# haberdashPI/SignalOperators.jl

Hardware: AMD Instinct MI355X
Metric: frames/sec sink() 44.1kHz 8ch Mix+Filt+Resample; achieved HBM GB/s (higher is better)
Workload: dtype f64

## Files before the change

signaloperators.jl_amd/csrc/executor.cpp:

```cpp
#include "plan_impl.h"

namespace so {

static inline int carrier_vec_ok(const DCarrier& c, int64_t V) {
    if (!std::getenv("SIGOPS_STRICT_ALIGN")) return (uintptr_t)c.base % (c.dtype == SO_F64 ? 8 : 4) == 0;
    return ((uintptr_t)c.base % 16 == 0) && (c.cstride % V == 0);
}

static hipError_t h2d_small(void* dst, const void* src, size_t bytes) {
    constexpr size_t kPiece = 16 * 1024;
    if (bytes < 2 * kPiece || bytes > (1u << 20)) return hipMemcpy(dst, src, bytes, hipMemcpyHostToDevice);
    for (size_t off = 0; off < bytes; off += kPiece) {
        const hipError_t e = hipMemcpy((char*)dst + off, (const char*)src + off, std::min(kPiece, bytes - off), hipMemcpyHostToDevice);
        if (e != hipSuccess) return e;
    }
    return hipSuccess;
}

static void upload_tables(Plan* P) {
    std::vector<Buf>& bufs = P->bufs;
    auto up = [&](int buf, const auto& v, size_t at = 0) {
        HIPCHECK(h2d_small((char*)bufs[buf].d + at, v.data(), v.size() * sizeof(*v.data())));
    };
    auto alloc_up = [](auto*& d, const auto& v) {
// ... 474 lines not shown
    g.src_has_omega = F.flag;
    g.src_df = F.df;
    g.src_omega = F.v0;
    g.src_phi = F.v1;
    g.src_fs = F.v2;
    const double step = 6.283185307179586476925 * (F.flag ? F.v0 / F.v2 : 1.0 / F.v2);
    g.src_cd = std::cos(step);
    g.src_sd = std::sin(step);
}
static RsGlobalTables global_tables(Plan* P, const Stage& S) {
    return RsGlobalTables{(const RsCtl*)P->bufs[S.ctl_buf].d, (const DCarrier*)P->bufs[S.car_buf].d, P->d_ops, P->d_leaves};
}
static void set_rsos_fixup(RsFixup& F, Plan* P, const Stage& S, const RsosItem& I) {
    F.g = I.g;
    F.tab = I.tab;
    F.jend = I.jend;
    F.jrel = (const int*)P->bufs[S.rsos_jrel_buf].d;
    F.taps = S.rsos_taps;
    F.cf = S.groups[0];
    F.gsrc = I.gsrc;
    F.y = I.y;
}
static void arm_bad(void* words, size_t n, hipStream_t st) { HIPCHECK((hipError_t)launch_fill_u32(words, n, 0x7f7f7f7fu, st)); }

static std::vector<long long> read_trace(const long long* d_trace, size_t trace_n, hipStream_t st, long long& t0) {
    std::vector<long long> tr(trace_n);
    HIPCHECK(hipStreamSynchronize(st));
    HIPCHECK(hipMemcpy(tr.data(), d_trace, trace_n * 8, hipMemcpyDeviceToHost));
    t0 = 0;
    for (size_t i = 0; i < trace_n; ++i)
        if (tr[i] && (!t0 || tr[i] < t0)) t0 = tr[i];
    return tr;
}
static void dump_rs_trace(const long long* d_trace, size_t trace_n, const RsPeriodic& rp, hipStream_t st) {
    long long t0;
    const std::vector<long long> tr = read_trace(d_trace, trace_n, st, t0);
    for (int w = 0; w < rp.nwaves; ++w)
        for (int it = 0; it < kRsTraceIters; ++it) {
            const long long* q = &tr[((size_t)w * kRsTraceIters + it) * kRsTraceStamps];
            if (!q[0]) continue;
            std::fprintf(stderr, "[rs-trace] %s w%02d it%02d", w < rp.ncompute ? "C" : "L", w, it);
            for (int k = 0; k < kRsTraceStamps; ++k) std::fprintf(stderr, " %lld", q[k] ? q[k] - t0 : -1);
            std::fprintf(stderr, "\n");
        }
}
static void dump_rsos_trace(const long long* d_trace, size_t trace_n, const RsSos& rs, hipStream_t st) {
    long long t0;
    const std::vector<long long> tr = read_trace(d_trace, trace_n, st, t0);
    const bool counters = std::atoi(std::getenv("SIGOPS_RSOS_TRACE")) == 2;
    for (int w = 0; w < rs.nwaves; ++w)
        for (int it = 0; it < (counters ? 5 : kRsosTraceIters); ++it) {
            const long long* q = &tr[((size_t)w * kRsosTraceIters + it) * 8];
            if (counters) {
                bool any = false;
                for (int k = 0; k < 8; ++k) any = any || q[k];
                if (!any) continue;
                std::fprintf(stderr, "[rsos-count] w%02d row%d", w, it);
                for (int k = 0; k < 8; ++k) std::fprintf(stderr, " %lld", q[k] - 1);
            } else {
                if (!q[0] && !q[2]) continue;
                std::fprintf(stderr, "[rsos-trace] %s w%02d it%02d", w == 0 ? "C" : (w & 3) == 0 ? "L" : "Y", w, it);
                for (int k = 0; k < 8; ++k) std::fprintf(stderr, " %lld", q[k] ? q[k] - t0 : -1);
            }
            std::fprintf(stderr, "\n");
        }
}


static int run_pointwise(Plan* P, const Step& s, void* outp, hipStream_t st) {
    const PwStep& w = P->pw[s.idx];
    if (w.nblocks <= 0) return 0;
    static const int il_scalar = std::getenv("SIGOPS_K1_ILSCALAR") ? 1 : 0;
    OutView ov{};
    if (w.out_buf >= 0) {
        const Buf& b = P->bufs[w.out_buf];
        ov = OutView{b.d, 1, b.pitch, b.dtype, il_scalar};
    } else if (P->out.is_device) {
        ov = OutView{outp, P->out.frame_stride, P->out.chan_stride, P->out.dtype, il_scalar};
    } else {
        const Buf& b = P->bufs[P->out_stage_buf];
        ov = OutView{b.d, P->interleaved_host ? P->out.nch : 1, P->interleaved_host ? 1 : b.pitch, b.dtype, il_scalar};
    }
    if (w.fill)
        launch_randn_fill(P->d_pieces + w.piece0, w.npieces, w.nblocks, P->d_leaves, ov, st);
    else if (w.rtc) {
        if (rtc_launch(w.rtc, w.nblocks, P->d_pieces + w.piece0, w.npieces, P->d_leaves, ov, st) != 0)
            fail(SO_ERR_RUNTIME, "hipRTC kernel launch failed");
    } else
// ... 251 lines not shown
    a.back = N.nd.l0;
    a.ahead = N.nd.l1;
    a.tab = S.aux_buf >= 0 ? (double*)P->bufs[S.aux_buf].d : nullptr;
    a.nch = N.nch;
    a.op = N.nd.i0;
    const int nl = launch_movsum(a, st);
    if (nl < 0) fail(SO_ERR_UNSUPPORTED, "Movsum: more than 65535 channels, or 2^31 tiles of 2048 frames or blocks of 1024 frames and more, are not lowered");
    return nl;
}

static int run_rsos_fused(Plan* P, const Stage& S, const SosGeom& g, const View& out, hipStream_t st) {
    const Node& N = P->nodes[S.node];
    const Stage& S3 = P->stages[S.rsos_src];
    RsSos rs = S.rs;
    rs.out_pitch = out.pitch;
    rs.out_f32 = g.out_dtype == SO_F32 || N.dtype == SO_F32;
    if (rs.f32m && rs.out_f32) rs.ring32 = 1;
    else rs.f32m = 0;
    rs.sring = rs.f32m && (rs.fuse == 1 || rs.fuse == 2) && !std::getenv("SIGOPS_RSOS_NO_SRING") ? 1 : 0;
    char* const yk = out.d - (size_t)S.rs.store_lo * (rs.out_f32 ? 4 : 8);
    rs.store_lo = S.rs.store_lo + g.store_lo;
    rs.mats = (const double*)P->bufs[S.rsos_mats_buf].d;
    rs.bad = nullptr;
    if (S.bad_buf >= 0 && rs.nranges >= 1 && !std::getenv("SIGOPS_SOS_NOPOISON")) {
        rs.bad = (int32_t*)P->bufs[S.bad_buf].d;
        arm_bad(rs.bad, (size_t)N.nch, st);
    }
    rs.err = kernel_error_word(P);
    static long long* d_rtrace = nullptr;
    static int rtrace_seen = 0;
    const char* const rtrace_skip = std::getenv("SIGOPS_RSOS_TRACE_SKIP");
    const bool rtracing = std::getenv("SIGOPS_RSOS_TRACE") != nullptr && rtrace_seen++ >= (rtrace_skip ? std::atoi(rtrace_skip) : 0);
    const size_t rtrace_n = (size_t)16 * kRsosTraceIters * 8;
    if (rtracing) {
        if (!d_rtrace) HIPCHECK(hipMalloc(&d_rtrace, rtrace_n * 8));
        HIPCHECK(hipMemsetAsync(d_rtrace, 0, rtrace_n * 8, st));
        rs.trace = d_rtrace;
    }
    const double* rtab = (const double*)P->bufs[S.rsos_tab_buf >= 0 ? S.rsos_tab_buf : S3.tab_buf].d;
    const int* rjend = (const int*)P->bufs[S.rsos_jend_buf >= 0 ? S.rsos_jend_buf : S3.jend_buf].d;
    if (launch_rsos(rtab, rjend, rs, yk, global_tables(P, S3), S.rsos_grid, st) != 0)
        fail(SO_ERR_RUNTIME, "internal: no fused resampler + IIR instantiation for this geometry");
    if (rtracing) dump_rsos_trace(d_rtrace, rtrace_n, rs, st);
    int nl = 1;
    if (rs.bad && S.rsos_jrel_buf >= 0 && !std::getenv("SIGOPS_RSOS_NO_FIXUP")) {
        RsFixup fx{};
        set_rsos_fixup(fx, P, S, RsosItem{rs, rtab, rjend, yk, global_tables(P, S3)});
        nl += launch_rsos_fixup(fx, st);
    } else if (rs.bad) {
        SosGeom pg = g;
        pg.n = rs.n_out;
        pg.chunk = rs.pr * rs.L;
        pg.nchunks = rs.nranges;
        pg.store_lo = rs.store_lo;
        pg.bad = rs.bad;
        nl += launch_sos_poison(yk, pg, st);
    }
    return nl;
}

static int run_sos(Plan* P, const Step& s, void* outp, hipStream_t st) {
    const Stage& S = P->stages[s.idx];
    const Node& N = P->nodes[S.node];
    const size_t esz = dsize(N.dtype);
    const View in = stage_in(P, S, N.nch, N.dtype), out = stage_out(P, s.idx, outp);
    SosGeom g = S.sg;
    g.in_pitch = in.pitch;
    g.out_pitch = out.pitch;
    g.store_lo = s.idx == P->alias_stage ? P->alias_skip : 0;
    if (s.idx == P->alias_stage && P->alias_narrow) g.out_dtype = SO_F32;
    g.align_rows = S.pre_stage < 0 && !std::getenv("SIGOPS_SOS_NOALIGN");
// ... 277 lines not shown
        if (!P->out.is_device && P->out.nframes > 0) {
            std::string why;
            if (kernel_gave_up(P, why)) fail(SO_ERR_RUNTIME, why);
        }
        if (P->profiling == 2) P->prof_execs++;
        if (P->profiling == 1) {
            HIPCHECK(hipStreamSynchronize(st));
            double total = 0, best = -1;
            for (size_t si = 0; si < P->steps.size(); ++si) {
                float ms = 0;
                HIPCHECK(hipEventElapsedTime(&ms, P->events[2 * si], P->events[2 * si + 1]));
                P->steps[si].ms = ms;
                total += ms;
                if (ms > best) {
                    best = ms;
                    P->stats.dominant_kernel_ms = ms;
                    P->stats.dominant_kernel_bytes = P->steps[si].bytes;
                    std::snprintf(P->stats.dominant_kernel, sizeof P->stats.dominant_kernel, "%s", P->steps[si].name.c_str());
                }
            }
            P->stats.last_exec_ms = total;
        }
    } catch (const PlanError& e) {
        err = e.msg;
        return e.status;
    }
    return SO_OK;
}

int plan_execute(Plan* P, void* outp, void* stream, std::string& err) {
    DeviceGuard guard(P->device);
    if (kernel_gave_up(P, err)) return SO_ERR_RUNTIME;
    const bool eligible = P->steps.size() >= 4 && P->out.is_device && P->host_leaves.empty() && !P->profiling &&
                          !std::getenv("SIGOPS_NO_GRAPH") && !std::getenv("SIGOPS_RS_TRACE");
    if (!eligible) {
        P->n_direct++;
        return plan_execute_direct(P, outp, stream, err);
    }
    hipStream_t st = (hipStream_t)stream;
    const bool leaves_match = P->out_alias_buf < 0 || P->bufs[P->out_alias_buf].d == outp;
    if (P->graph_exec && P->graph_out == outp && P->graph_epoch == P->array_epoch && leaves_match) {
        if (hipSetDevice(P->device) == hipSuccess && hipGraphLaunch(P->graph_exec, st) == hipSuccess) {
            P->n_replays++;
            return SO_OK;
        }
        (void)hipGetLastError();
        (void)hipGraphExecDestroy(P->graph_exec);
        P->graph_exec = nullptr;
        P->graph_failed = true;
    }
    if (P->graph_failed || P->last_out != outp || P->last_epoch != P->array_epoch) {
        P->last_out = outp;
        P->last_epoch = P->array_epoch;
        P->n_direct++;
        return plan_execute_direct(P, outp, stream, err);
    }
    if (P->graph_exec && P->graph_out == outp && P->graph_epoch == P->array_epoch) {
// ... 175 lines not shown
```

signaloperators.jl_amd/csrc/k_exact.hip:

```cpp
#include "kcommon.h"
#include "kstage.h"

namespace so {

constexpr int kFixThreads = 256;
constexpr int kFixSeg = 1024;
constexpr int kFixIn = 6144;
constexpr int kFixAhead = 64;

template <typename TO>
__device__ __forceinline__ void rsos_fixup_body(const RsFixup& fx) {
    const RsSos& g = fx.g;
    const int ch = blockIdx.y;
    if (ch >= g.nch) return;
    const int r = g.bad[ch];
    if (r < 0 || r >= g.nranges) return;
    TO* const y = (TO*)fx.y + (int64_t)ch * g.out_pitch;
    const int64_t prL = g.pr * g.L;
    const double nan = __longlong_as_double(0x7ff8000000000000ll);
    {
        int64_t f0 = (int64_t)(r + 1) * prL;
        if (f0 < g.store_lo) f0 = g.store_lo;
        for (int64_t f = f0 + (int64_t)blockIdx.x * kFixThreads + threadIdx.x; f < g.n_out; f += (int64_t)gridDim.x * kFixThreads) y[f] = (TO)nan;
    }
    if (blockIdx.x != 0) return;
    __shared__ long long s_first;
    __shared__ double xin[kFixIn];
    __shared__ double xs[kFixSeg];
    __shared__ double ys[kFixAhead + 16];
    const int tid = threadIdx.x;
    const int64_t lo = max((int64_t)r * prL, g.store_lo), hi = min((int64_t)(r + 1) * prL, g.n_out);
    if (tid == 0) s_first = hi;
    __syncthreads();
    for (int64_t m = lo + tid; m < hi; m += kFixThreads)
        if (!isfinite((double)y[m])) {
            atomicMin(&s_first, (long long)m);
            break;
// ... 161 lines not shown
```

signaloperators.jl_amd/csrc/k_rsos.hip:

```cpp
#include "kcommon.h"
#include "kstage.h"

#ifndef SO_RSOS_ONLY_KS
#define SO_RSOS_ONLY_KS -1
#endif
#ifndef SO_RSOS_ONLY_F32
#define SO_RSOS_ONLY_F32 0
#endif
#ifndef SO_RSOS_ONLY_NW
#define SO_RSOS_ONLY_NW 0
#endif

namespace so {

typedef double v4d __attribute__((ext_vector_type(4)));
typedef float v4f __attribute__((ext_vector_type(4)));

#define SO_LDS __attribute__((address_space(3)))
__device__ __forceinline__ int flag_ld(uint32_t a) { return *(const volatile SO_LDS int*)(uintptr_t)a; }
__device__ __forceinline__ void flag_st(uint32_t a, int v) { *(volatile SO_LDS int*)(uintptr_t)a = v; }
#define SO_SPIN_PAUSE(spins, sleep, limit)                         \
    do {                                                           \
        if (++(spins) > (limit)) rsos_wait_failed(sh);             \
        if ((sleep) == 1) __builtin_amdgcn_s_sleep(1);             \
// ... 207 lines not shown
};

__device__ __forceinline__ int uni(int v) { return __builtin_amdgcn_readfirstlane(v); }


#define SO_GLB __attribute__((address_space(1)))

__device__ __forceinline__ void rsos_wait_failed(SO_LDS RsosShared* sh) {
    uint32_t SO_GLB* const e = (uint32_t SO_GLB*)rfl64((int64_t)(uintptr_t)sh->g.err);
    if (e == nullptr) __builtin_trap();
    if ((threadIdx.x & 63) == 0) __hip_atomic_store((uint32_t*)e, 1u, __ATOMIC_RELAXED, __HIP_MEMORY_SCOPE_SYSTEM);
    __threadfence_system();
    asm volatile("s_waitcnt vmcnt(0) lgkmcnt(0)" ::: "memory");
    __builtin_amdgcn_endpgm();
}

#ifndef SO_RSOS_TRACE
#define SO_RSOS_TRACE 0
#endif
__device__ __forceinline__ void rsos_stamp(long long* trace, int wave, int it, int k, int it0 = 400) {
    if constexpr (!SO_RSOS_TRACE) return;
    if (trace != nullptr && blockIdx.x == 0 && (threadIdx.x & 63) == 0 && it >= it0 && it < it0 + kRsosTraceIters)
        ((long long SO_GLB*)trace)[(wave * kRsosTraceIters + (it - it0)) * 8 + k] = clock64();
}

#ifndef SO_RSOS_COUNT
#define SO_RSOS_COUNT 0
#endif
__device__ __forceinline__ void rsos_count_out(long long* trace, int wave, int row, int k, long long v) {
    if constexpr (!SO_RSOS_COUNT) return;
    if (trace != nullptr && blockIdx.x == 0) ((long long SO_GLB*)trace)[((wave * kRsosTraceIters) + row) * 8 + k] = v + 1;
}

struct RsosLds {
    SO_LDS double *taps, *ring, *gtab;
    volatile SO_LDS double *xs, *ss;
    volatile SO_LDS double* xh;
};
__device__ __forceinline__ SO_LDS double* rsos_lds_ptr(const void* p) {
    return (SO_LDS double*)(uintptr_t)__builtin_amdgcn_readfirstlane((uint32_t)(uintptr_t)(const SO_LDS void*)p);
}
#ifndef SO_NSS_EXTRA
#define SO_NSS_EXTRA (ny + 1)
#endif
__host__ __device__ constexpr int rsos_nss(int ny) { return ny + SO_NSS_EXTRA; }
__device__ __forceinline__ RsosLds rsos_carve(double* dyn_, int tapd, int rpitch, int nx, int ns) {
// ... 697 lines not shown
    if (g.store_lo > r0 * g.pr * g.L) return false;
    const int64_t lo_ok = C0.a > 0 ? C0.a : 0, hi_ok = C0.b < g.n_in ? C0.b : g.n_in;
    const int64_t f0 = (r0 * g.pr - g.wp) * g.M + g.wj0, f1 = (r1 * g.pr - g.wp) * g.M + g.wj0 + g.wk;
    return f0 >= lo_ok && f1 <= hi_ok;
}

template <int NY>
__device__ __attribute__((noinline)) void rsos_wproj_y(RsosShared* sh_, double* dyn, int64_t G_, int yi_) {
    constexpr int NX = 2 * NY + 1;
    const int lane = threadIdx.x & 63;
    SO_LDS RsosShared* const sh = (SO_LDS RsosShared*)rsos_lds_ptr(sh_);
    const int64_t G = rfl64(G_);
    const int yi = uni(yi_);
    const SO_LDS RsSos& g = sh->g;
    const RsosLds l = rsos_carve(dyn, uni(g.cyc) > 0 ? 0 : uni(g.ngroups) * uni(g.ks) * 64, uni(g.rpitch), NX, rsos_nss(NY));
    const uint32_t fl_base = (uint32_t)(uintptr_t)sh->flags;
    const int ct = uni(g.ct), K = uni(g.wk);
    const int npairs = (K + 7) >> 3;
    const int c0 = (int)((int64_t)yi * npairs / NY), c1 = (int)((int64_t)(yi + 1) * npairs / NY);
    const double SO_GLB* const V = (const double SO_GLB*)rfl64((int64_t)(uintptr_t)g.mats) + 14 * 64 + lane;
    const SO_LDS DCarrier& C0 = sh->ctl.car[0];
    const int64_t ncg = uni(g.nch) / ct;
    const int gq = lane >> 4, n16 = lane & 15;
    const int64_t r = (G / ncg) * uni(g.rgs) + n16 / ct;
    const int64_t f0 = (r * rfl64(g.pr) - uni(g.wp)) * rfl64(g.M) + uni(g.wj0);
    const double SO_GLB* const row = (const double SO_GLB*)rfl64((int64_t)(uintptr_t)C0.base) +
                                     ((int64_t)((int)(G % ncg) * ct + n16 % ct) * rfl64(C0.cstride) + rfl64(C0.df) + f0 + 2 * gq);
    v4d acc = v4d{0.0, 0.0, 0.0, 0.0};
    auto mm = [&](const double (&a)[16], const v2d (&b)[8]) __attribute__((always_inline)) {
#pragma unroll
        for (int i = 0; i < 8; ++i) {
            acc = __builtin_amdgcn_mfma_f64_16x16x4f64(a[2 * i], b[i][0], acc, 0, 0, 0);
            acc = __builtin_amdgcn_mfma_f64_16x16x4f64(a[2 * i + 1], b[i][1], acc, 0, 0, 0);
        }
    };
    auto load = [&](int c, double (&a)[16], v2d (&b)[8]) __attribute__((always_inline)) {
        const double SO_GLB* const vp = V + (size_t)c * 128;
        const double SO_GLB* const rp = row + (size_t)c * 8;
#pragma unroll
        for (int i = 0; i < 8; ++i) {
            a[2 * i] = vp[i * 128];
            a[2 * i + 1] = vp[i * 128 + 64];
            b[i] = *(const v2d_a8 SO_GLB*)(rp + 8 * i);
        }
    };
    double aA[16], aB[16];
    v2d bA[8], bB[8];
    const int c1f = min(c1, K >> 3);
    const int nfull = c1f > c0 ? (c1f - c0) >> 3 : 0;
    if (nfull > 0) {
        load(c0, aA, bA);
        for (int n = 0; n < nfull; n += 2) {
            const int c = c0 + 8 * n;
            if (n + 1 < nfull) load(c + 8, aB, bB);
            mm(aA, bA);
            if (n + 2 < nfull) load(c + 16, aA, bA);
            if (n + 1 < nfull) mm(aB, bB);
        }
    }
    {
        const int c = c0 + 8 * nfull;
#pragma unroll
        for (int i = 0; i < 8; ++i) {
            const int cc = c + i;
            aA[2 * i] = aA[2 * i + 1] = 0.0;
            bA[i] = v2d{0.0, 0.0};
            if (cc < c1) {
                aA[2 * i] = V[(size_t)(2 * cc) * 64];
                aA[2 * i + 1] = V[(size_t)(2 * cc + 1) * 64];
                const int f = 8 * cc + 2 * gq;
                if (f + 1 < K) bA[i] = *(const v2d_a8 SO_GLB*)(row + 8 * cc);
                else if (f < K) bA[i][0] = row[8 * cc];
            }
        }
        mm(aA, bA);
    }
#pragma unroll
    for (int v = 0; v < 3; ++v) l.ss[(1 + yi) * 192 + v * 64 + lane] = acc[v];
    flag_st(fl_base + 4 * (kRsosFlagWp + yi), 1);
}

template <int NY>
__device__ __attribute__((noinline)) void rsos_wproj_chain(RsosShared* sh_, double* dyn, int64_t G_) {
    constexpr int NX = 2 * NY + 1;
    const int lane = threadIdx.x & 63;
    SO_LDS RsosShared* const sh = (SO_LDS RsosShared*)rsos_lds_ptr(sh_);
    const int64_t G = rfl64(G_);
    const SO_LDS RsSos& g = sh->g;
    const RsosLds l = rsos_carve(dyn, uni(g.cyc) > 0 ? 0 : uni(g.ngroups) * uni(g.ks) * 64, uni(g.rpitch), NX, rsos_nss(NY));
    const uint32_t fl_base = (uint32_t)(uintptr_t)sh->flags;
    const int ct = uni(g.ct), fuse = uni(g.fuse);
    const int gq = lane >> 4, n16 = lane & 15;
    double s[3] = {0.0, 0.0, 0.0};
    if (fuse >= 0) {
        const SO_LDS DCarrier& C0 = sh->ctl.car[0];
        const DLeaf leaf0 = leaf_uniform(sh_->ctl.leaves[min(kCtlLeaves - 1, max(0, uni(C0.slot_leaf[0])))]);
        const int64_t ncg = uni(g.nch) / ct;
        const int64_t r = (G / ncg) * uni(g.rgs) + n16 / ct;
        const int64_t f0 = (r * rfl64(g.pr) - uni(g.wp)) * rfl64(g.M) + uni(g.wj0);
        const double2 sc = rsos_sine_at(f0 + leaf0.df + 1, leaf0.v0, leaf0.v1, leaf0.v2, leaf0.flag);
        const double SO_GLB* const W = (const double SO_GLB*)rfl64((int64_t)(uintptr_t)g.mats) + 14 * 64 + (size_t)((uni(g.wk) + 7) >> 3) * 128;
#pragma unroll
        for (int v = 0; v < 3; ++v) {
            const double t = fma(sc.y, W[gq + 4 * v], sc.x * W[16 + gq + 4 * v]);
            s[v] = fuse == 2 ? -t : t;
        }
    }
    int spins = 0;
    for (;;) {
        const int f = lane < NY ? flag_ld(fl_base + 4 * (kRsosFlagWp + lane)) : 1;
        if (wave_min(f, NY) >= 1) break;
        SO_SPIN_PAUSE(spins, 1, 1 << 22);
    }
#pragma unroll
    for (int yi = 0; yi < NY; ++yi)
#pragma unroll
        for (int v = 0; v < 3; ++v) s[v] += l.ss[(1 + yi) * 192 + v * 64 + lane];
#pragma unroll
    for (int v = 0; v < 3; ++v) l.ss[v * 64 + lane] = s[v];
}

template <int NY>
__device__ __attribute__((noinline)) void rsos_helper(RsosShared* sh_, double* dyn) {
    constexpr int NX = 2 * NY + 1;
    const int lane = threadIdx.x & 63;
    SO_LDS RsosShared* const sh = (SO_LDS RsosShared*)rsos_lds_ptr(sh_);
    const SO_LDS RsSos& g = sh->g;
    const RsosLds l = rsos_carve(dyn, 0, uni(g.rpitch), NX, rsos_nss(NY));
    const int NB = (uni(sh->wpe) + (int)rfl64(g.pr)) * uni(g.ngroups);
    const double SO_GLB* mats = (const double SO_GLB*)rfl64((int64_t)(uintptr_t)g.mats);
    const uint32_t fl_base = (uint32_t)(uintptr_t)sh->flags;
    const int debug = uni(g.debug);
    const bool f32m = uni(g.f32m) != 0 && uni(g.out_f32) != 0;
    double Dk[4];
#pragma unroll
    for (int v = 0; v < 4; ++v) Dk[v] = f32m ? mats[(lane >> 4) * 64 + v * 16 + (lane & 15)] : mats[v * 64 + lane];
    __builtin_amdgcn_s_setprio(1);
    constexpr int res[3] = {kRsosHres0, kRsosHres1, kRsosHres2};
    int hslot[3] = {kRsosHres0 % NX, kRsosHres1 % NX, kRsosHres2 % NX}, hring = 0;
    for (int b0 = 0; b0 < NB; b0 += NY) {
#pragma unroll
        for (int j = 0; j < 3; ++j) {
// ... 60 lines not shown
#pragma unroll
    for (int v = 0; v < 4; ++v) Tk[v] = F32M ? mats[(7 + (lane >> 4)) * 64 + v * 16 + (lane & 15)] : mats[(7 + v) * 64 + lane];
#pragma unroll
    for (int v = 0; v < 3; ++v) Ck[v] = mats[(11 + v) * 64 + lane];
    int cl;
    int nb0;
    {
        const int ri = n16 / ct;
        cl = ((grp.e0m + ri * grp.prMm) & 15) + gq;
        const int64_t ob = grp.ob0 + ri * grp.prL;
        nb0 = ob < 0 ? (int)((-ob) / 16) : 0;
    }
    const SO_LDS char* const ringc = (const SO_LDS char*)l.ring + (uint32_t)n16 * (uint32_t)rpitch * 8u;
    uint32_t yo0;
    int64_t ystep[4];
    const int64_t ybase_e = (int64_t)(grp.cg * ct) * out_pitch + grp.ob0;
#ifndef SO_Y_EARLY
#define SO_Y_EARLY 0
#endif
#ifndef SO_Y_SADDR
#define SO_Y_SADDR 1
#endif
#ifndef SO_ST_NT
#define SO_ST_NT ""
#endif
    const bool yfits = SO_Y_SADDR && uni((int)((((int64_t)(ct - 1) * out_pitch + (int64_t)(16 / ct) * grp.prL + 16) * (int64_t)sizeof(TO)) < ((int64_t)1 << 32)));
    int nbs_all;
    {
        int m = 0x7fffffff;
        int64_t off0 = 0;
#pragma unroll
        for (int v = 0; v < 4; ++v) {
            const int row = gq + 4 * v;
            const int ri = row / ct, cv = row % ct;
            const int64_t ob = grp.ob0 + ri * grp.prL;
            const int64_t off = ((int64_t)cv * out_pitch + (int64_t)ri * grp.prL + n16) * (int64_t)sizeof(TO);
            if (v == 0) off0 = off;
            ystep[v] = rfl64(off - off0);
            const int64_t tl = n_out - ob - n16;
            const int64_t nb = tl <= 0 ? 0 : (tl + 15) / 16;
            m = min(m, (int)(nb > 0x3fffffff ? 0x3fffffff : nb));
        }
        yo0 = (uint32_t)off0;
#pragma unroll
        for (int off = 32; off > 0; off >>= 1) m = min(m, __shfl_xor(m, off, 64));
        nbs_all = uni(m);
    }
// ... 72 lines not shown
        if (pb_ >= nbl_max && pb_ < nbs_all) {
#pragma unroll
            for (int v = 0; v < 4; ++v) put(v, (TO)ay[v]);
        } else {
#pragma unroll
            for (int v = 0; v < 4; ++v) {
                const int64_t m = out_index(v);
                if (m >= slo && m < n_out) put(v, (TO)ay[v]);
            }
        }
    };
    auto back = [&](int sq, double (&sv)[3], v4d& pay_) __attribute__((always_inline)) {
        back_wait(sq, sv);
        if (ppi_ < wp) return;
        rsos_stamp(trace, wave, pb_ / NY, 4, 40);
        back_store(back_mfma(sv, pay_), true);
        rsos_stamp(trace, wave, pb_ / NY, 5, 40);
    };
    using TapT = std::conditional_t<F32M, float, double>;
    auto block = [&](int b, const TapT (&at)[KS], v4d& pin, v4d& pout, int je, int jn) __attribute__((always_inline)) {
        const int wb = pi * M + je - ulo_kw;
        const int need = wb + kw + 16;
        rsos_stamp(trace, wave, b / NY, 0, 40);
        int spins = 0;
        if constexpr (SO_RSOS_COUNT) cnt_in_b += avail < need ? 1 : 0;
        while (avail < need && !(debug & 16)) {
            const int v = lane < NL ? flag_ld(fl_base + 4 * (kRsosFlagLdp + lane)) : 0x7fffffff;
            avail = wave_min(v, NL);
            if (avail < need) {
                SO_SPIN_PAUSE(spins, 2, 1 << 22);
                if constexpr (SO_RSOS_COUNT) ++cnt_in;
            }
        }
        rsos_stamp(trace, wave, b / NY, 1, 40);
        int sq = 0;
        double sv[3] = {0.0, 0.0, 0.0};
        if (pb_ >= 0) {
            sq = flag_ld(f_sseq);
#pragma unroll
            for (int v = 0; v < 3; ++v) sv[v] = l.ss[pslot_ * 192 + v * 64 + lane];
        }
        if (wbm < 0) wbm = wb % RING;
        const int pos = wbm + cl;
        double bx[KS];
        bool have_bx = false;
        [[maybe_unused]] float bf32[KS];
// ... 186 lines not shown
            for (int s = 0; s < KS; ++s) at[s] = tp[s * 64];
            int gn = gi + NY;
            while (gn >= ngroups) gn -= ngroups;
            const int je = uni(sh->jend[gi]), jn = uni(sh->jend[gn]);
            if (cur == 0) block(b, at, payA, payB, je, jn);
            else block(b, at, payB, payA, je, jn);
            cur ^= 1;
        }
        last_back();
    }
}


constexpr int rsos_nthreads(int nw) { return (nw == 17 ? 16 : nw) * 64; }
template <int KS, int NW, typename TO, int CYC>
__device__ __forceinline__ void rsos_body(const double* __restrict__ tab, const int* __restrict__ jend_g, const RsSos& g, TO* __restrict__ y,
                                          const RsGlobalTables& gsrc, int64_t G0, int64_t Gstep) {
    constexpr bool HW = NW == 17;
    constexpr int NT = rsos_nthreads(NW);
    constexpr int NY = NW >= 16 ? 10 : NW - 2, NL = NW == 16 ? 2 : 1, NX = 2 * NY + 1;
    extern __shared__ double lds_raw[];
    __shared__ RsosShared sh;
    const int wave = uni(threadIdx.x >> 6);
    {
        if (threadIdx.x == 0) {
            sh.g = g;
            sh.gcar = gsrc.car;
            sh.gops = gsrc.ops;
            sh.gleaves = gsrc.leaves;
            sh.y = (void*)y;
            sh.tab = tab;
        }
    }
    if constexpr (CYC == 0)
        for (int i = threadIdx.x; i < g.ngroups * KS * 64; i += NT) lds_raw[i] = tab[i];
    for (int i = threadIdx.x; i < g.ngroups; i += NT) sh.jend[i] = jend_g[i];
    {
        const int* src = reinterpret_cast<const int*>(gsrc.ctl);
        int* dst = reinterpret_cast<int*>(&sh.ctl);
        for (int i = threadIdx.x; i < (int)(sizeof(RsCtl) / 4); i += NT) dst[i] = src[i];
    }
    const int64_t ncg = g.nch / g.ct;
    const int64_t ngrp = ncg * ((g.nranges + g.rgs - 1) / g.rgs);
    double* const ss = lds_raw + (CYC > 0 ? 0 : (size_t)g.ngroups * KS * 64) + (size_t)16 * g.rpitch + (size_t)NX * 192;
    const int ru = g.ct < 8 ? g.ct : 8;
    for (int64_t G = G0; G < ngrp; G += Gstep) {
        __syncthreads();
        if (threadIdx.x < kRsosFlags) sh.flags[threadIdx.x] = 0;
        if (threadIdx.x < 192) ss[threadIdx.x] = 0.0;
        if (threadIdx.x == 0) {
            const bool pj = NW != 16 && NW != 17 && rsos_wproj_group(sh, G);
            sh.proj = pj ? 1 : 0;
            sh.wpe = pj ? 0 : g.wp;
            if (pj) sh.flags[kRsosFlagSseq] = -1;
        }
        __syncthreads();
        const bool proj = sh.proj != 0;
        if (wave == 0) {
            if (!(g.debug & 64)) {
                if (proj) rsos_wproj_chain<NY>(&sh, lds_raw, G);
                const int nk = (g.debug & 131072) ? 3 : (2 * g.nsec + 3) / 4;
                if (nk <= 1) rsos_chain<NY, 1>(&sh, lds_raw, G);
                else if (nk == 2) rsos_chain<NY, 2>(&sh, lds_raw, G);
                else rsos_chain<NY, 3>(&sh, lds_raw, G);
            }
        } else if (NW == 16 && (wave == 13 || wave == 14)) {
            if (!g.gsplit || (g.debug & 256) || g.src32) continue;
            const int q = wave - 13;
            if (g.arr2) {
                if constexpr (NL == 2) {
                    if (ru == 8) rsos_loader<NY, NL, 8, false, 0, 2, true>(&sh, lds_raw, G, q);
                    else if (ru == 4) rsos_loader<NY, NL, 4, false, 0, 2, true>(&sh, lds_raw, G, q);
                    else if (ru == 2) rsos_loader<NY, NL, 2, false, 0, 2, true>(&sh, lds_raw, G, q);
                }
            } else if (ru == 2) {
                if (g.rpitch == 770) rsos_loader<NY, NL, 2, false, 770 * 8, 2>(&sh, lds_raw, G, q);
                else if (g.rpitch == 642) rsos_loader<NY, NL, 2, false, 642 * 8, 2>(&sh, lds_raw, G, q);
                else rsos_loader<NY, NL, 2, false, 0, 2>(&sh, lds_raw, G, q);
            } else if (ru == 4) {
                if (g.rpitch == 770) rsos_loader<NY, NL, 4, false, 770 * 8, 2>(&sh, lds_raw, G, q);
// ... 233 lines not shown
```

signaloperators.jl_amd/csrc/plan_impl.h:

```cpp
#pragma once
#include <hip/hip_runtime.h>

#include <algorithm>
#include <chrono>
#include <cmath>
#include <cstdio>
#include <cstdlib>
#include <cstring>
#include <map>
#include <memory>
#include <mutex>
#include <set>
#include <string>
#include <vector>

#include "kernels.h"
#include "plan.h"
#include "sigops_internal.h"

namespace so {


struct PlanError {
    int status;
// ... 87 lines not shown
    int64_t norm_df = 0;
    int out_buf = -1, in_buf = -1, aux_buf = -1;
    int64_t win_off = -1;
    const void* in_ptr = nullptr;
    int in_array_node = -1;
    int64_t in_offset = 0;
    int64_t in_pitch = 0, in_frames = 0;
    int pw_step = -1;
    int pos_buf = -1, pos_array_node = -1, pos_pw_step = -1;
    int64_t pos_offset = 0, pos_pitch = 0;
    int64_t x_fstride = 1;
    std::vector<DCarrier> carriers;
    int car_buf = -1;
    int ctl_buf = -1;
    std::vector<SosCoefs> groups;
    SosGeom sg{};
    int mpow_buf = -1, v_buf = -1, s0_buf = -1;
    int src_op = 0;
    DLeaf src_fn{};
    bool xscan = false;
    int batch = -1;
    int xs_mats_buf = -1, sblk_buf = -1;
    int bad_buf = -1;
    std::vector<std::vector<double>> xs_mats_host;
    std::vector<std::vector<double>> mpow_host;
    size_t mpow_stride() const {
        size_t n = 0;
        for (auto& v : mpow_host) n = std::max(n, v.size());
        return n;
    }
    bool onepass = false;
    SosOne so1{};
    int one_tabs_buf = -1, one_sync_buf = -1, one_vpub_buf = -1;
    std::vector<double> one_tabs_host;
    std::vector<size_t> one_tabs_off;
    RsGeom rg{};
    int pfb_buf = -1, dpfb_buf = -1;
    std::vector<double> pfb_host, dpfb_host;
    bool periodic = false;
    RsPeriodic rp{};
    bool tiled = false;
    RsTiled rt{};
    std::vector<double> rsos_tab_host;
    std::vector<int> rsos_jend_host;
    int rsos_tab_buf = -1, rsos_jend_buf = -1;
    int rsb = -1;
// ... 129 lines not shown
    void try_window_alias(std::vector<Piece>& rootp);
    int alias_stage = -1;
    bool alias_narrow = false;
    int64_t alias_skip = 0;
    bool interleaved_host = false;
    std::vector<char> host_tmp;
    int profiling = 0;
    int64_t prof_execs = 0;
    std::vector<hipEvent_t> events;
    std::vector<std::vector<int>> step_deps;
    std::vector<int> step_lane;
    std::vector<char> step_signals;
    int nlanes = 1;
    std::vector<hipStream_t> lane_streams;
    std::vector<hipEvent_t> step_done;
    hipEvent_t ev_start = nullptr;
    void plan_lanes();
    hipGraphExec_t graph_exec = nullptr;
    hipStream_t capture_stream = nullptr;
    const void* graph_out = nullptr;
    const void* last_out = nullptr;
    int64_t array_epoch = 0, graph_epoch = -1, last_epoch = -1;
    bool graph_failed = false;
    int64_t n_replays = 0, n_captures = 0, n_direct = 0;
    so_stats_t stats{};
    int64_t algo_bytes = 0;
    std::map<int, bool> array_counted;

    int add_expr(const Expr& e) {
        exprs.push_back(e);
        return (int)exprs.size() - 1;
    }
    int new_buf(int64_t frames, int nch, int dtype) {
        Buf b;
        b.frames = frames;
        b.pitch = (frames + 63) / 64 * 64;
        if (b.pitch == 0) b.pitch = 64;
        b.nch = nch;
        b.dtype = dtype;
        b.bytes = (size_t)b.pitch * (size_t)std::max(nch, 1) * dsize(dtype);
        bufs.push_back(b);
        return (int)bufs.size() - 1;
    }
    int raw_buf(size_t bytes) {
        Buf b;
        b.bytes = std::max<size_t>(bytes, 8);
// ... 202 lines not shown
```

signaloperators.jl_amd/csrc/sigops_internal.h:

```cpp
#pragma once
#include <cstdint>

namespace so {

enum OpCode : int32_t {
    OP_CONST = 0,
    OP_LOAD = 1,
    OP_SCALAR = 2,
    OP_FUNC = 3,
    OP_RAMP = 4,
    OP_ADD = 5,
    OP_SUB = 6,
    OP_MUL = 7,
    OP_DIV = 8,
    OP_NEG = 9,
    OP_ROUND32 = 10,
    OP_STOREF = 11,
    OP_LOADF = 12
};

enum LeafMode : int32_t { LM_PLAIN = 0, LM_CYCLE = 1, LM_MIRROR = 2 };

struct DOp {
    int32_t code;
// ... 288 lines not shown
    int64_t out_pitch;
    int64_t store_lo;
    const double* mats;
    int32_t* bad;
    long long* trace;
    uint32_t* err;
};
constexpr int kRsosTraceIters = 96;

struct RsosItem {
    RsSos g;
    const double* tab;
    const int* jend;
    void* y;
    RsGlobalTables gsrc;
};

struct RsFixup {
    RsSos g;
    const double* tab;
    const int* jend;
    const int* jrel;
    int32_t taps;
    int32_t pad;
    SosCoefs cf;
    RsGlobalTables gsrc;
    void* y;
};

struct RsRows {
    int64_t n_in, n_out;
    int64_t L, M;
    int64_t nperiods;
    int32_t taps;
    int32_t ct, pb;
    int32_t jlo;
    int32_t tile_len;
    int32_t pitch;
    int32_t nch;
    int32_t debug;
    int32_t kw, ngroups, pbshift;
    int32_t threads;
    int64_t in_pitch, out_pitch;
};

}
```

signaloperators.jl_amd/csrc/stages.cpp:

```cpp
#include "plan_impl.h"

namespace so {

static int env_int(const char* name, int dflt) {
    const char* ev = std::getenv(name);
    return ev ? std::atoi(ev) : dflt;
}

constexpr size_t kRsLdsAvail = 160 * 1024 - sizeof(RsCtl) - 64;

static int channels_per_group(int nch, int max) {
    if (max >= 16 && nch % 16 == 0) return 16;
    for (int c : {8, 4, 2})
        if (nch % c == 0) return c;
    return 1;
}


struct Tap {
    double hv, dv;
};
static Tap tap(const double* h, int hlen, int nphi, int p, int64_t age) {
    const int64_t hi = p + (int64_t)nphi * age;
    return {hi < hlen ? h[hi] : 0.0, hi + 1 < hlen ? h[hi + 1] - h[hi] : 0.0};
// ... 348 lines not shown
    stages[sid].groups = groups;
    stages[sid].mpow_host = mp;
    if (nchunks > 1 && !stages[sid].onepass) {
        size_t msz = 0;
        for (auto& v : mp) msz = std::max(msz, v.size());
        stages[sid].mpow_buf = sized_buf(stages[sid].mpow_buf, msz * 8 * groups.size());
        stages[sid].v_buf = sized_buf(stages[sid].v_buf, (size_t)nchunks * nch * 2 * kMaxSec * 8);
        stages[sid].s0_buf = sized_buf(stages[sid].s0_buf, (size_t)nchunks * nch * 2 * kMaxSec * 8);
        if (xscan) {
            stages[sid].xscan = true;
            stages[sid].xs_mats_host.clear();
            for (auto& cf : groups) {
                const int D = 2 * cf.nsec;
                Mat M = matpow(sos_state_matrix(cf), L, D), MB = matpow(M, kXsBlock, D);
                std::vector<double> both(M);
                both.insert(both.end(), MB.begin(), MB.end());
                stages[sid].xs_mats_host.push_back(both);
            }
            stages[sid].xs_mats_buf = sized_buf(stages[sid].xs_mats_buf, (size_t)groups.size() * 2 * 16 * 16 * 8);
            const int64_t nblk = (nchunks + kXsBlock - 1) / kXsBlock;
            stages[sid].sblk_buf = sized_buf(stages[sid].sblk_buf, (size_t)nblk * nch * 16 * 8);
        }
    }
    if (nchunks > 1 && !stages[sid].onepass && !exact) stages[sid].bad_buf = sized_buf(stages[sid].bad_buf, (size_t)nch * 4);
    stages[sid].sg = g;
}

static bool plain_load(const Expr& e, int dtype, int nch, bool unit_stride, bool strict_pitch) {
    const DLeaf& l = e.leaf;
    if (e.op != E_LOAD || l.mode != LM_PLAIN || l.sf != 1 || l.sc != 1 || l.dtype != dtype || l.df < 0 || l.dc < 0) return false;
    if (unit_stride ? l.fstride != 1 : l.fstride < 1) return false;
    return l.cstride > 0 || (l.cstride == -1 && (!strict_pitch || (e.array_node < 0 && l.dc == 0))) || nch == 1;
}
static int64_t leaf_offset(const DLeaf& l) { return l.df * l.fstride + l.dc * std::max<int64_t>(l.cstride, 0); }

void Plan::stage_input(int sid, const std::vector<Piece>& ps, int64_t frames, int nch, int dtype) {
    Stage& S = stages[sid];
    S.in_frames = frames;
    if (ps.size() == 1 && plain_load(exprs[ps[0].e], dtype, ps[0].r.c1 - ps[0].r.c0, false, true)) {
        const Expr& e = exprs[ps[0].e];
        S.in_array_node = e.array_node;
        S.in_buf = e.array_node >= 0 ? -1 : e.leaf.buf;
        S.x_fstride = e.leaf.fstride;
        S.in_pitch = e.leaf.cstride;
        S.in_offset = e.array_node >= 0 ? leaf_offset(e.leaf) : e.leaf.df * e.leaf.fstride;
        if (e.array_node >= 0) count_array(e.array_node);
        return;
// ... 1762 lines not shown
                        const long double cs = cosl(2.0L * 3.141592653589793238462643383279502884L * ph);
                        for (int i = 0; i < 12; ++i) {
                            vs[i] += (long double)V[(size_t)i * K + f] * sn;
                            vc[i] += (long double)V[(size_t)i * K + f] * cs;
                        }
                    }
                    for (int i = 0; i < 12; ++i) {
                        mt[(size_t)14 * 64 + (size_t)K8 / 4 * 64 + i] = (double)vs[i];
                        mt[(size_t)14 * 64 + (size_t)K8 / 4 * 64 + 16 + i] = (double)vc[i];
                    }
                }
                S2.rs.wproj = 1;
                S2.rs.wk = K;
                S2.rs.wj0 = j0;
                if (std::getenv("SIGOPS_DEBUG_PLAN"))
                    std::fprintf(stderr, "[sigops] k_rsos: warm-up as one product: %d frames from %d (%d k-steps instead of %lld blocks)\n", K, j0, K8 / 4,
                                 (long long)(wp * ngp));
            }
        }
    }

    void commit_launch() {
        S2.rsos_mats_buf = P.raw_buf(S2.rsos_mats_host.size() * 8);
        if (S2.bad_buf < 0) S2.bad_buf = P.raw_buf((size_t)nch * 4);
        S3.fused_away = true;
        if (alt.armed) {
            alt.armed = false;
            P.bufs[S3.in_buf].bytes = 0;
        }
        if (std::getenv("SIGOPS_DEBUG_PLAN"))
            std::fprintf(stderr,
                         "[sigops] resampler + IIR fused (k_rsos): %lld ranges of %lld periods (+%lld warm-up), %lld groups of %d ch x %d ranges, "
                         "ks=%d ring=%d chunk=%d waves=%d cyc=%d fuse=%d/%d\n",
                         (long long)nranges, (long long)pr, (long long)wp, (long long)ngrp, ct, rgs, ks, g.ring, g.chunk, g.nwaves, g.cyc,
                         g.fuse, g.fuse_sine);
    }
};

void Plan::fuse_resample_sos() {
    if (std::getenv("SIGOPS_NO_RSOS")) return;
    for (size_t i2 = 0; i2 < stages.size(); ++i2) {
        Stage& S2 = stages[i2];
        if (S2.kind != ST_SOS || S2.onepass || S2.need <= 0 || S2.groups.size() != 1 || S2.groups[0].nsec > 6 ||
            S2.in_buf < 0 || S2.in_array_node >= 0 || S2.in_offset != S2.base || S2.pw_step >= 0 || S2.sg.exact || (S2.xscan && !S2.under_norm) ||
            (S2.under_norm && (S2.norm_df != 0 || S2.base != 0 || std::getenv("SIGOPS_NORM_EXACT_FILT"))) || S2.src_op || S2.batch >= 0 || S2.pre_stage >= 0 ||
            (nodes[S2.node].dtype != SO_F64 && nodes[S2.node].dtype != SO_F32) || S2.in_frames != S2.need - S2.base)
            continue;
// ... 130 lines not shown
};

void Plan::fuse_plain_sos() {
    if (std::getenv("SIGOPS_NO_RSOS") || std::getenv("SIGOPS_NO_PLAIN_RSOS")) return;
    const int cus = env_int("SIGOPS_RSOS_GRID", 256);
    const PlainRsos one{*this, nodes, stages, cus};
    int candidates = 0;
    for (auto& S : stages)
        if (S.kind == ST_SOS && S.rsos_src < 0 && S.carriers.size() == 1 && S.need > 0) ++candidates;
    std::vector<size_t> small;
    for (size_t i2 = 0; i2 < stages.size(); ++i2) {
        Stage& S2 = stages[i2];
        if (S2.kind != ST_SOS || S2.rsos_src >= 0 || S2.carriers.size() != 1 || S2.need <= 0 || S2.onepass || S2.sg.exact || (S2.xscan && !S2.under_norm) ||
            (S2.under_norm && S2.norm_df != 0) || S2.batch >= 0 || S2.pre_stage >= 0 || S2.base != 0 || S2.groups.size() != 1 || S2.groups[0].nsec > 6 || S2.pw_step >= 0)
            continue;
        if (candidates > 1 && (int64_t)S2.need * nodes[S2.node].nch < ((int64_t)1 << 26) && !std::getenv("SIGOPS_RSOS_MINGROUPS")) {
            small.push_back(i2);
            continue;
        }
        RsSos g{};
        double cost = 0.0;
        if (!one.fit(i2, 0, g, cost)) continue;
        one.commit(i2, g);
        if (S2.bad_buf < 0) S2.bad_buf = raw_buf((size_t)g.nch * 4);
    }
    const char* const want_s = std::getenv("SIGOPS_RSOS_BATCH");
    const int want = want_s && *want_s ? std::atoi(want_s) : -1;
    if (small.size() < 2 || want == 0) return;
    std::map<std::pair<int, int>, std::vector<size_t>> kinds;
    for (size_t i2 : small) {
        if ((int)i2 == alias_stage) continue;
        {
            const DCarrier& c0 = stages[i2].carriers[0];
            bool plain = c0.array_node >= 0 && c0.buf < 0;
            for (int k = 0; k < c0.nslots && plain; ++k)
                if (leaves[c0.slot_leaf[k]].buf >= 0) plain = false;
            if (!plain) continue;
        }
        RsSos g{};
        double cost = 0.0;
        if (!one.fit(i2, 1 << 20, g, cost)) continue;
        kinds[{nodes[stages[i2].node].dtype == SO_F32 ? 1 : 0, g.nwaves}].push_back(i2);
    }
    for (auto& kv : kinds) {
        const std::vector<size_t>& cand = kv.second;
        if (cand.size() < 2) continue;
        const int gpm = (int)std::max<int64_t>(1, cus / (int64_t)cand.size());
// ... 161 lines not shown
```

Baseline: 30.02 billion.

## Double-buffer rsos poison words and rearm them in the fixup kernel

The bad-range poison buffer is doubled to two sets. The fixup kernel now re-poisons the spare set for the next call, which removes the separate fill launch on each non-graph execution. Output stores also default to non-temporal, and extra prologue trace stamps are added under the trace flag. This adds mutable per-stage state that must be reset on errors and when graph capture is used.

Result: faster. 30.33 billion (median of 6 runs) (+1.0%).

```diff
diff --git a/signaloperators.jl_amd/csrc/executor.cpp b/signaloperators.jl_amd/csrc/executor.cpp
--- a/signaloperators.jl_amd/csrc/executor.cpp
+++ b/signaloperators.jl_amd/csrc/executor.cpp
@@ -520,6 +520,9 @@
     F.y = I.y;
 }
 static void arm_bad(void* words, size_t n, hipStream_t st) { HIPCHECK((hipError_t)launch_fill_u32(words, n, 0x7f7f7f7fu, st)); }
+static void disarm_bad(Plan* P) {
+    for (const Stage& S : P->stages) S.bad_armed = false;
+}
 
 static std::vector<long long> read_trace(const long long* d_trace, size_t trace_n, hipStream_t st, long long& t0) {
     std::vector<long long> tr(trace_n);
@@ -562,6 +565,12 @@
             }
             std::fprintf(stderr, "\n");
         }
+    for (int w = 0; w < rs.nwaves && w < 16 && !counters; ++w) {
+        const long long* q = &tr[((size_t)16 * kRsosTraceIters + w) * 8];
+        std::fprintf(stderr, "[rsos-trace-pro] w%02d", w);
+        for (int k = 0; k < 8; ++k) std::fprintf(stderr, " %lld", q[k] ? q[k] - t0 : -1);
+        std::fprintf(stderr, "\n");
+    }
 }
 
 
@@ -859,16 +868,30 @@
     rs.store_lo = S.rs.store_lo + g.store_lo;
     rs.mats = (const double*)P->bufs[S.rsos_mats_buf].d;
     rs.bad = nullptr;
+    const bool fixup = S.rsos_jrel_buf >= 0 && !std::getenv("SIGOPS_RSOS_NO_FIXUP");
+    int rearm = 0;
     if (S.bad_buf >= 0 && rs.nranges >= 1 && !std::getenv("SIGOPS_SOS_NOPOISON")) {
-        rs.bad = (int32_t*)P->bufs[S.bad_buf].d;
-        arm_bad(rs.bad, (size_t)N.nch, st);
+        int32_t* const words = (int32_t*)P->bufs[S.bad_buf].d;
+        const size_t nch = (size_t)N.nch;
+        if (fixup && !P->graph_plan && rs.nch == N.nch && P->bufs[S.bad_buf].bytes >= 2 * nch * 4) {
+            if (!S.bad_armed) {
+                arm_bad(words, 2 * nch, st);
+                S.bad_set = 0;
+            }
+            rs.bad = words + (S.bad_set ? nch : 0);
+            rearm = S.bad_set ? -(int)nch : (int)nch;
+        } else {
+            S.bad_armed = false;
+            rs.bad = words;
+            arm_bad(rs.bad, nch, st);
+        }
     }
     rs.err = kernel_error_word(P);
     static long long* d_rtrace = nullptr;
     static int rtrace_seen = 0;
     const char* const rtrace_skip = std::getenv("SIGOPS_RSOS_TRACE_SKIP");
     const bool rtracing = std::getenv("SIGOPS_RSOS_TRACE") != nullptr && rtrace_seen++ >= (rtrace_skip ? std::atoi(rtrace_skip) : 0);
-    const size_t rtrace_n = (size_t)16 * kRsosTraceIters * 8;
+    const size_t rtrace_n = (size_t)(16 * kRsosTraceIters + 16) * 8;
     if (rtracing) {
         if (!d_rtrace) HIPCHECK(hipMalloc(&d_rtrace, rtrace_n * 8));
         HIPCHECK(hipMemsetAsync(d_rtrace, 0, rtrace_n * 8, st));
@@ -880,10 +903,15 @@
         fail(SO_ERR_RUNTIME, "internal: no fused resampler + IIR instantiation for this geometry");
     if (rtracing) dump_rsos_trace(d_rtrace, rtrace_n, rs, st);
     int nl = 1;
-    if (rs.bad && S.rsos_jrel_buf >= 0 && !std::getenv("SIGOPS_RSOS_NO_FIXUP")) {
+    if (rs.bad && fixup) {
         RsFixup fx{};
         set_rsos_fixup(fx, P, S, RsosItem{rs, rtab, rjend, yk, global_tables(P, S3)});
+        fx.rearm = rearm;
         nl += launch_rsos_fixup(fx, st);
+        if (rearm != 0) {
+            S.bad_set ^= 1;
+            S.bad_armed = true;
+        }
     } else if (rs.bad) {
         SosGeom pg = g;
         pg.n = rs.n_out;
@@ -1207,6 +1235,7 @@
             P->stats.last_exec_ms = total;
         }
     } catch (const PlanError& e) {
+        disarm_bad(P);
         err = e.msg;
         return e.status;
     }
@@ -1215,9 +1244,13 @@
 
 int plan_execute(Plan* P, void* outp, void* stream, std::string& err) {
     DeviceGuard guard(P->device);
-    if (kernel_gave_up(P, err)) return SO_ERR_RUNTIME;
+    if (kernel_gave_up(P, err)) {
+        disarm_bad(P);
+        return SO_ERR_RUNTIME;
+    }
     const bool eligible = P->steps.size() >= 4 && P->out.is_device && P->host_leaves.empty() && !P->profiling &&
                           !std::getenv("SIGOPS_NO_GRAPH") && !std::getenv("SIGOPS_RS_TRACE");
+    P->graph_plan = eligible;
     if (!eligible) {
         P->n_direct++;
         return plan_execute_direct(P, outp, stream, err);
diff --git a/signaloperators.jl_amd/csrc/k_exact.hip b/signaloperators.jl_amd/csrc/k_exact.hip
--- a/signaloperators.jl_amd/csrc/k_exact.hip
+++ b/signaloperators.jl_amd/csrc/k_exact.hip
@@ -13,6 +13,7 @@
     const RsSos& g = fx.g;
     const int ch = blockIdx.y;
     if (ch >= g.nch) return;
+    if (fx.rearm != 0 && blockIdx.x == 0 && threadIdx.x == 0) g.bad[ch + fx.rearm] = 0x7f7f7f7f;
     const int r = g.bad[ch];
     if (r < 0 || r >= g.nranges) return;
     TO* const y = (TO*)fx.y + (int64_t)ch * g.out_pitch;
diff --git a/signaloperators.jl_amd/csrc/k_rsos.hip b/signaloperators.jl_amd/csrc/k_rsos.hip
--- a/signaloperators.jl_amd/csrc/k_rsos.hip
+++ b/signaloperators.jl_amd/csrc/k_rsos.hip
@@ -253,6 +253,13 @@
     if constexpr (!SO_RSOS_TRACE) return;
     if (trace != nullptr && blockIdx.x == 0 && (threadIdx.x & 63) == 0 && it >= it0 && it < it0 + kRsosTraceIters)
         ((long long SO_GLB*)trace)[(wave * kRsosTraceIters + (it - it0)) * 8 + k] = clock64();
+}
+__device__ __forceinline__ void rsos_stamp_pro(long long* trace, int k) {
+    if constexpr (!SO_RSOS_TRACE) return;
+    if (trace != nullptr && blockIdx.x == 1 && (threadIdx.x & 63) == 0) {
+        long long SO_GLB* const q = (long long SO_GLB*)trace + ((16 * kRsosTraceIters + (int)(threadIdx.x >> 6)) * 8 + k);
+        if (*q == 0) *q = clock64();
+    }
 }
 
 #ifndef SO_RSOS_COUNT
@@ -996,6 +1003,9 @@
     const SO_LDS DCarrier& C0 = sh->ctl.car[0];
     const int64_t ncg = uni(g.nch) / ct;
     const int gq = lane >> 4, n16 = lane & 15;
+    long long* trace = nullptr;
+    if constexpr (SO_RSOS_TRACE) trace = (long long*)rfl64((int64_t)(uintptr_t)g.trace);
+    rsos_stamp_pro(trace, 0);
     const int64_t r = (G / ncg) * uni(g.rgs) + n16 / ct;
     const int64_t f0 = (r * rfl64(g.pr) - uni(g.wp)) * rfl64(g.M) + uni(g.wj0);
     const double SO_GLB* const row = (const double SO_GLB*)rfl64((int64_t)(uintptr_t)C0.base) +
@@ -1024,6 +1034,10 @@
     const int nfull = c1f > c0 ? (c1f - c0) >> 3 : 0;
     if (nfull > 0) {
         load(c0, aA, bA);
+        if constexpr (SO_RSOS_TRACE) {
+            asm volatile("s_waitcnt vmcnt(0)" ::: "memory");
+            rsos_stamp_pro(trace, 1);
+        }
         for (int n = 0; n < nfull; n += 2) {
             const int c = c0 + 8 * n;
             if (n + 1 < nfull) load(c + 8, aB, bB);
@@ -1032,6 +1046,7 @@
             if (n + 1 < nfull) mm(aB, bB);
         }
     }
+    rsos_stamp_pro(trace, 2);
     {
         const int c = c0 + 8 * nfull;
 #pragma unroll
@@ -1047,11 +1062,16 @@
                 else if (f < K) bA[i][0] = row[8 * cc];
             }
         }
+        if constexpr (SO_RSOS_TRACE) {
+            asm volatile("s_waitcnt vmcnt(0)" ::: "memory");
+            rsos_stamp_pro(trace, 3);
+        }
         mm(aA, bA);
     }
 #pragma unroll
     for (int v = 0; v < 3; ++v) l.ss[(1 + yi) * 192 + v * 64 + lane] = acc[v];
     flag_st(fl_base + 4 * (kRsosFlagWp + yi), 1);
+    rsos_stamp_pro(trace, 4);
 }
 
 template <int NY>
@@ -1066,6 +1086,9 @@
     const int ct = uni(g.ct), fuse = uni(g.fuse);
     const int gq = lane >> 4, n16 = lane & 15;
     double s[3] = {0.0, 0.0, 0.0};
+    long long* trace = nullptr;
+    if constexpr (SO_RSOS_TRACE) trace = (long long*)rfl64((int64_t)(uintptr_t)g.trace);
+    rsos_stamp_pro(trace, 0);
     if (fuse >= 0) {
         const SO_LDS DCarrier& C0 = sh->ctl.car[0];
         const DLeaf leaf0 = leaf_uniform(sh_->ctl.leaves[min(kCtlLeaves - 1, max(0, uni(C0.slot_leaf[0])))]);
@@ -1086,12 +1109,14 @@
         if (wave_min(f, NY) >= 1) break;
         SO_SPIN_PAUSE(spins, 1, 1 << 22);
     }
+    rsos_stamp_pro(trace, 1);
 #pragma unroll
     for (int yi = 0; yi < NY; ++yi)
 #pragma unroll
         for (int v = 0; v < 3; ++v) s[v] += l.ss[(1 + yi) * 192 + v * 64 + lane];
 #pragma unroll
     for (int v = 0; v < 3; ++v) l.ss[v * 64 + lane] = s[v];
+    rsos_stamp_pro(trace, 2);
 }
 
 template <int NY>
@@ -1198,7 +1223,7 @@
 #define SO_Y_SADDR 1
 #endif
 #ifndef SO_ST_NT
-#define SO_ST_NT ""
+#define SO_ST_NT " nt"
 #endif
     const bool yfits = SO_Y_SADDR && uni((int)((((int64_t)(ct - 1) * out_pitch + (int64_t)(16 / ct) * grp.prL + 16) * (int64_t)sizeof(TO)) < ((int64_t)1 << 32)));
     int nbs_all;
@@ -1317,6 +1342,7 @@
         const int wb = pi * M + je - ulo_kw;
         const int need = wb + kw + 16;
         rsos_stamp(trace, wave, b / NY, 0, 40);
+        rsos_stamp_pro(trace, 5);
         int spins = 0;
         if constexpr (SO_RSOS_COUNT) cnt_in_b += avail < need ? 1 : 0;
         while (avail < need && !(debug & 16)) {
@@ -1549,6 +1575,7 @@
     extern __shared__ double lds_raw[];
     __shared__ RsosShared sh;
     const int wave = uni(threadIdx.x >> 6);
+    rsos_stamp_pro(g.trace, 6);
     {
         if (threadIdx.x == 0) {
             sh.g = g;
@@ -1583,6 +1610,7 @@
         }
         __syncthreads();
         const bool proj = sh.proj != 0;
+        rsos_stamp_pro(g.trace, 7);
         if (wave == 0) {
             if (!(g.debug & 64)) {
                 if (proj) rsos_wproj_chain<NY>(&sh, lds_raw, G);
diff --git a/signaloperators.jl_amd/csrc/plan_impl.h b/signaloperators.jl_amd/csrc/plan_impl.h
--- a/signaloperators.jl_amd/csrc/plan_impl.h
+++ b/signaloperators.jl_amd/csrc/plan_impl.h
@@ -133,6 +133,8 @@
     int batch = -1;
     int xs_mats_buf = -1, sblk_buf = -1;
     int bad_buf = -1;
+    mutable int bad_set = 0;
+    mutable bool bad_armed = false;
     std::vector<std::vector<double>> xs_mats_host;
     std::vector<std::vector<double>> mpow_host;
     size_t mpow_stride() const {
@@ -308,6 +310,7 @@
     const void* last_out = nullptr;
     int64_t array_epoch = 0, graph_epoch = -1, last_epoch = -1;
     bool graph_failed = false;
+    bool graph_plan = false;
     int64_t n_replays = 0, n_captures = 0, n_direct = 0;
     so_stats_t stats{};
     int64_t algo_bytes = 0;
diff --git a/signaloperators.jl_amd/csrc/sigops_internal.h b/signaloperators.jl_amd/csrc/sigops_internal.h
--- a/signaloperators.jl_amd/csrc/sigops_internal.h
+++ b/signaloperators.jl_amd/csrc/sigops_internal.h
@@ -334,7 +334,7 @@
     const int* jend;
     const int* jrel;
     int32_t taps;
-    int32_t pad;
+    int32_t rearm;
     SosCoefs cf;
     RsGlobalTables gsrc;
     void* y;
diff --git a/signaloperators.jl_amd/csrc/stages.cpp b/signaloperators.jl_amd/csrc/stages.cpp
--- a/signaloperators.jl_amd/csrc/stages.cpp
+++ b/signaloperators.jl_amd/csrc/stages.cpp
@@ -394,7 +394,7 @@
             stages[sid].sblk_buf = sized_buf(stages[sid].sblk_buf, (size_t)nblk * nch * 16 * 8);
         }
     }
-    if (nchunks > 1 && !stages[sid].onepass && !exact) stages[sid].bad_buf = sized_buf(stages[sid].bad_buf, (size_t)nch * 4);
+    if (nchunks > 1 && !stages[sid].onepass && !exact) stages[sid].bad_buf = sized_buf(stages[sid].bad_buf, (size_t)nch * 8);
     stages[sid].sg = g;
 }
 
@@ -2203,7 +2203,7 @@
 
     void commit_launch() {
         S2.rsos_mats_buf = P.raw_buf(S2.rsos_mats_host.size() * 8);
-        if (S2.bad_buf < 0) S2.bad_buf = P.raw_buf((size_t)nch * 4);
+        if (S2.bad_buf < 0) S2.bad_buf = P.raw_buf((size_t)nch * 8);
         S3.fused_away = true;
         if (alt.armed) {
             alt.armed = false;
@@ -2380,7 +2380,7 @@
         double cost = 0.0;
         if (!one.fit(i2, 0, g, cost)) continue;
         one.commit(i2, g);
-        if (S2.bad_buf < 0) S2.bad_buf = raw_buf((size_t)g.nch * 4);
+        if (S2.bad_buf < 0) S2.bad_buf = raw_buf((size_t)g.nch * 8);
     }
     const char* const want_s = std::getenv("SIGOPS_RSOS_BATCH");
     const int want = want_s && *want_s ? std::atoi(want_s) : -1;
```
